# Scoobadood/TSDF

Hardware: AMD Instinct MI355X
Metric: Mvoxels/s integrate + Mrays/s raycast, 512^3 grid, 640x480 depth; 1/2/4/8 GPU (higher is better)
Workload: dtype f32; 1 GPU; configs[2]: 512^3 TSDF over 3000 mm, synthetic TUM-surrogate stream (200-frame trajectory, seed 0x5EED0003), 640x480 uint16 depth, bilateral(30,4.5) + integrate + raycast + normals per frame; parallelism=zslab1, depth_tile_maxima=left by the bilateral filter's launch, ranks=1

## Files before the change

### include/tsdf_amd.h

```cpp
#ifndef TSDF_AMD_H
#define TSDF_AMD_H

#include <stddef.h>
#include <stdint.h>

#ifdef __cplusplus
extern "C" {
#endif

#define TSDF_OK 0
#define TSDF_ERR_INVALID 1
#define TSDF_ERR_DEVICE 2
#define TSDF_ERR_NOMEM 3

typedef struct tsdf_volume tsdf_volume;
typedef struct tsdf_bilateral tsdf_bilateral;
typedef struct tsdf_icp tsdf_icp;

typedef struct tsdf_volume_info {
    uint32_t size[3];
    uint32_t z_begin, z_end;
    uint32_t z_store_begin, z_store_end;
    float physical_size[3];
    float voxel_size[3];
// ... 31 lines not shown
                            tsdf_volume **out);
int tsdf_volume_destroy(tsdf_volume *volume);
int tsdf_volume_set_stream(tsdf_volume *volume, void *hip_stream);
int tsdf_volume_stream(const tsdf_volume *volume, void **hip_stream);
int tsdf_volume_synchronize(const tsdf_volume *volume);
int tsdf_volume_clear(tsdf_volume *volume);
int tsdf_volume_get_info(const tsdf_volume *volume, tsdf_volume_info *info);
int tsdf_volume_set_offset(tsdf_volume *volume, float ox, float oy, float oz);

int tsdf_volume_set_header(tsdf_volume *volume, const float offset[3], float truncation_distance,
                           float max_weight, const float global_translation[3],
                           const float global_rotation[3]);

int tsdf_volume_distances(const tsdf_volume *volume, float **device_ptr);
int tsdf_volume_mark_dirty(tsdf_volume *volume);
int tsdf_volume_weights(const tsdf_volume *volume, float **device_ptr);
int tsdf_volume_weight_storage(const tsdf_volume *volume, int *bits_per_weight, int *pinned);
int tsdf_volume_set_weight_storage(tsdf_volume *volume, int bits_per_weight);
int tsdf_selftest_count_division(uint32_t b_begin, uint32_t b_end, unsigned long long *mismatches);
int tsdf_selftest_bilateral_chain_taps(size_t n, const float *w, const uint32_t *v4, const float *s, float *s_f32, float *s_f64,
                                       uint8_t *certified);
int tsdf_selftest_bilateral_chain_image(float sigma_colour, float sigma_space, const void *image, int bits_per_pixel, int width, int height,
                                        void *filtered, unsigned long long counts[4]);
int tsdf_volume_deformation(tsdf_volume *volume, tsdf_deformation_node **device_ptr);
int tsdf_volume_set_distance_data(tsdf_volume *volume, const float *host);
int tsdf_volume_set_weight_data(tsdf_volume *volume, const float *host);
int tsdf_volume_set_deformation(tsdf_volume *volume, const tsdf_deformation_node *host);
int tsdf_volume_deform_points(const tsdf_volume *volume, int num_points, float *host_points);
int tsdf_volume_deform_points_device(const tsdf_volume *volume, int num_points, float *device_points);
int tsdf_volume_get_distance_data(const tsdf_volume *volume, float *host);
int tsdf_volume_get_weight_data(const tsdf_volume *volume, float *host);
int tsdf_volume_get_deformation_planes(const tsdf_volume *volume, uint32_t plane_begin, uint32_t plane_count,
                                       tsdf_deformation_node *host);
int tsdf_volume_set_offset_at_clear(tsdf_volume *volume, const float offset_at_clear[3]);

int tsdf_integrate(tsdf_volume *volume, const uint16_t *host_depth, uint32_t width, uint32_t height,
                   const float pose[16], const float inv_pose[16], const float k[9], const float kinv[9]);
int tsdf_integrate_device(tsdf_volume *volume, const uint16_t *device_depth, uint32_t width,
                          uint32_t height, const float pose[16], const float inv_pose[16],
                          const float k[9], const float kinv[9]);
int tsdf_integrate_device_tiles(tsdf_volume *volume, const uint16_t *device_depth, uint32_t width,
                                uint32_t height, const float pose[16], const float inv_pose[16],
                                const float k[9], const float kinv[9], const uint16_t *device_tile_max);
int tsdf_integrate_prepare_device_tiles(tsdf_volume *volume, const uint16_t *device_depth, uint32_t width,
                                        uint32_t height, const float pose[16], const float inv_pose[16],
                                        const float k[9], const float kinv[9], const uint16_t *device_tile_max,
// ... 316 lines not shown
```

### tsdf_amd/_capi.py

```python
import ctypes as C
import os

_HERE = os.path.dirname(os.path.abspath(__file__))
LIB_PATH = os.environ.get("TSDF_HIP_LIB") or os.path.join(_HERE, "lib", "libtsdf_hip.so")

TSDF_OK, TSDF_ERR_INVALID, TSDF_ERR_DEVICE, TSDF_ERR_NOMEM = 0, 1, 2, 3
TSDF_FIELD_UNIT_GRADIENT = 1
TSDF_RAYS_BAND_ONLY = 1
TSDF_MESH_NORMALS, TSDF_MESH_COLOURS = 1, 2
TSDF_MESH_KEEP_LARGEST = 1
TSDF_SMOOTH_PIN_BOUNDARY, TSDF_SMOOTH_NORMALS = 1, 2
TSDF_ESDF_FILL_UNKNOWN = 1
TSDF_SCENE_FLOW_DEFORMED = 1


class TsdfError(RuntimeError):
    """A C-ABI call failed with TSDF_ERR_DEVICE / TSDF_ERR_NOMEM."""


class VolumeInfo(C.Structure):
    _fields_ = [("size", C.c_uint32 * 3), ("z_begin", C.c_uint32), ("z_end", C.c_uint32),
                ("z_store_begin", C.c_uint32), ("z_store_end", C.c_uint32),
                ("physical_size", C.c_float * 3), ("voxel_size", C.c_float * 3), ("offset", C.c_float * 3),
                ("offset_at_clear", C.c_float * 3), ("truncation_distance", C.c_float),
# ... 60 lines not shown
    "tsdf_stream_synchronize": (_i, [_vp]),
    "tsdf_volume_create": (_i, [_u32, _u32, _u32, _f, _f, _f, C.POINTER(_vp)]),
    "tsdf_volume_create_slab": (_i, [_u32, _u32, _u32, _f, _f, _f, _u32, _u32, C.POINTER(_vp)]),
    "tsdf_volume_destroy": (_i, [_vp]),
    "tsdf_volume_set_stream": (_i, [_vp, _vp]),
    "tsdf_volume_stream": (_i, [_vp, C.POINTER(_vp)]),
    "tsdf_volume_synchronize": (_i, [_vp]),
    "tsdf_volume_clear": (_i, [_vp]),
    "tsdf_volume_get_info": (_i, [_vp, C.POINTER(VolumeInfo)]),
    "tsdf_volume_set_offset": (_i, [_vp, _f, _f, _f]),
    "tsdf_volume_set_header": (_i, [_vp, _fp, _f, _f, _fp, _fp]),
    "tsdf_volume_mark_dirty": (_i, [_vp]),
    "tsdf_volume_distances": (_i, [_vp, C.POINTER(_vp)]),
    "tsdf_volume_weights": (_i, [_vp, C.POINTER(_vp)]),
    "tsdf_volume_weight_storage": (_i, [_vp, C.POINTER(_i), C.POINTER(_i)]),
    "tsdf_volume_last_raycast_kind": (_i, [_vp, C.POINTER(_i)]),
    "tsdf_volume_last_cell_list": (_i, [_vp, C.POINTER(C.c_uint32)]),
    "tsdf_volume_set_weight_storage": (_i, [_vp, _i]),
    "tsdf_volume_set_weight_cap": (_i, [_vp, C.c_uint32]),
    "tsdf_volume_weight_cap": (_i, [_vp, C.POINTER(C.c_uint32)]),
    "tsdf_selftest_count_division": (_i, [_u32, _u32, C.POINTER(C.c_uint64)]),
    "tsdf_selftest_bilateral_chain_taps": (_i, [C.c_size_t, _vp, _vp, _vp, _vp, _vp, _vp]),
    "tsdf_selftest_bilateral_chain_image": (_i, [_f, _f, _vp, _i, _i, _i, _vp, C.POINTER(C.c_uint64)]),
    "tsdf_volume_deformation": (_i, [_vp, C.POINTER(_vp)]),
    "tsdf_volume_set_distance_data": (_i, [_vp, _vp]),
    "tsdf_volume_set_weight_data": (_i, [_vp, _vp]),
    "tsdf_volume_set_deformation": (_i, [_vp, _vp]),
    "tsdf_volume_get_distance_data": (_i, [_vp, _vp]),
    "tsdf_measure_copy_bandwidth": (_i, [C.c_size_t, _i, _vp, C.POINTER(C.c_double)]),
    "tsdf_measure_update_bandwidth": (_i, [_i, _vp, C.POINTER(C.c_double)]),
    "tsdf_volume_get_weight_data": (_i, [_vp, _vp]),
    "tsdf_volume_get_deformation_planes": (_i, [_vp, C.c_uint32, C.c_uint32, _vp]),
    "tsdf_volume_set_offset_at_clear": (_i, [_vp, _vp]),
    "tsdf_integrate": (_i, [_vp, _vp, _u32, _u32, _fp, _fp, _fp, _fp]),
    "tsdf_integrate_device": (_i, [_vp, _vp, _u32, _u32, _fp, _fp, _fp, _fp]),
    "tsdf_deintegrate": (_i, [_vp, _vp, _u32, _u32, _fp, _fp, _fp, _fp]),
    "tsdf_deintegrate_device": (_i, [_vp, _vp, _u32, _u32, _fp, _fp, _fp, _fp]),
    "tsdf_integrate_device_tiles": (_i, [_vp, _vp, _u32, _u32, _fp, _fp, _fp, _fp, _vp]),
    "tsdf_integrate_prepare_device_tiles": (_i, [_vp, _vp, _u32, _u32, _fp, _fp, _fp, _fp, _vp, _vp]),
    "tsdf_integrate_discard_prepared": (_i, [_vp]),
    "tsdf_volume_set_timing": (_i, [_vp, _i]),
    "tsdf_volume_kernel_time": (_i, [_vp, _i, C.POINTER(C.c_uint32), C.POINTER(C.c_float)]),
    "tsdf_volume_set_counting": (_i, [_vp, _i]),
    "tsdf_volume_last_updated_voxels": (_i, [_vp, C.POINTER(C.c_uint64)]),
    "tsdf_volume_last_distance_stores": (_i, [_vp, C.POINTER(C.c_uint64)]),
    "tsdf_volume_enable_colour": (_i, [_vp, _i]),
# ... 190 lines not shown
```

### tsdf_amd/csrc/raycast.hip

```cpp
#include <algorithm>
#include <cmath>
#include <cstdlib>

#include "common.hpp"
#include "raycast_sample.hpp"
#include "field_sample.hpp"

namespace tsdf {

__device__ inline bool can_intersect_in_dimension(float space_min, float space_max, float origin, float direction,
                                                  float &near_t, float &far_t) {
    bool can_intersect = true;
    if (direction == 0) {
        if (origin < space_min || origin > space_max) can_intersect = false;
    } else {
        float dmin = (space_min - origin) / direction;
        float dmax = (space_max - origin) / direction;
        if (dmin > dmax) {
            float t = dmin;
            dmin = dmax;
            dmax = t;
        }
        if (dmin > near_t) near_t = dmin;
        if (dmax < far_t) far_t = dmax;
        if (near_t > far_t) can_intersect = false;
        else if (far_t < 0) can_intersect = false;
    }
    return can_intersect;
}
// ... 202 lines not shown
    }

    k_first = k_lo;
    if (SLAB && k_end > 0) {
        const float za = ((float)rp.own_lo - 2.0f) * g.vs.z, zb = ((float)rp.own_hi + 2.0f) * g.vs.z;
        if (dir.z != 0.0f) {
            const float r = __builtin_amdgcn_rcpf(dir.z);
            const float t0 = (za - sz) * r, t1 = (zb - sz) * r;
            const float ta = fminf(t0, t1), tb = fmaxf(t0, t1);
            const float ka = floorf(ta * __builtin_amdgcn_rcpf(step_size)) - 3.0f;
            const float kb = ceilf(tb * __builtin_amdgcn_rcpf(step_size)) + 3.0f;
            if (ka > (float)k_first) k_first = (int)fminf(ka, (float)kMaxSamples);
            if (kb < (float)k_end) k_end = (int)fmaxf(kb, 0.0f);
        } else if (sz < za || sz > zb) {
            k_end = 0;
        }
    }
}

__device__ inline SkipCtx make_skip_ctx(const Geom &g, float step_size) {
    SkipCtx sc;
    sc.inv_vx = __builtin_amdgcn_rcpf(g.vs.x); sc.inv_vy = __builtin_amdgcn_rcpf(g.vs.y); sc.inv_vz = __builtin_amdgcn_rcpf(g.vs.z);
    sc.inv_step = __builtin_amdgcn_rcpf(step_size);
    sc.eps = fmaxf(1.0e-3f, 2.0e-6f * (float)max(g.X, max(g.Y, g.Z)));
    sc.tx = sc.ty = sc.tz = INFINITY;
    sc.su = sc.sv = sc.sw = INFINITY;
    sc.posx = sc.posy = sc.posz = 1.0f;
    sc.skip_ok = false;
    return sc;
}

struct TailQueue {
    uint2 *entries;
    uint32_t *count;
    uint32_t trip_budget;
    uint32_t lanes;
    uint64_t *best;
    int piece_min;
    const uint32_t *order;
    uint8_t *heavy;
    uint32_t heavy_passes;
};
constexpr uint32_t kTailSignals = 4 + 2 * 256;
constexpr uint32_t kNoHit = 0xffffffffu;
constexpr uint32_t kNoSlot = 0xffffffffu;
__host__ __device__ inline uint32_t ray_range_of_slot(uint32_t z, uint32_t nz, uint32_t order) {
    return order == 0 ? z : order == 1 ? nz - 1u - z : (z == 0 ? nz - 1u : z == 1 ? 0u : nz - z);
// ... 875 lines not shown
                          nullptr);
}

int tsdf_volume_cast_rays_colour_device(const tsdf_volume *v, uint64_t n, const float *device_origins, const float *device_directions,
                                        const float *device_t_max, float *device_points, float *device_t, float *device_normals,
                                        uint8_t *device_rgb) {
    int rc = cast_rays_colour_check(v, n, device_origins, device_directions, device_points, device_t, device_normals, device_rgb);
    if (rc != TSDF_OK) return rc;
    if (n == 0) return TSDF_OK;
    rc = cast_rays(const_cast<tsdf_volume *>(v), n, device_origins, device_directions, device_t_max, device_points, device_t, device_normals);
    if (rc != TSDF_OK) return rc;
    return cast_rays_colour(v, n, device_points, device_rgb);
}

int tsdf_volume_cast_rays_colour(const tsdf_volume *cv, uint64_t n, const float *host_origins, const float *host_directions,
                                 const float *host_t_max, float *host_points, float *host_t, float *host_normals, uint8_t *host_rgb) {
    const int rc0 = cast_rays_colour_check(cv, n, host_origins, host_directions, host_points, host_t, host_normals, host_rgb);
    if (rc0 != TSDF_OK) return rc0;
    if (n == 0) return TSDF_OK;
    return cast_rays_host(const_cast<tsdf_volume *>(cv), n, host_origins, host_directions, host_t_max, host_points, host_t, host_normals,
                          host_rgb);
}

}
```

### tsdf_amd/csrc/raycast_cells.hpp

```cpp

struct RayRecord {
    float near_t;
    uint32_t k_range;
};
static_assert(sizeof(RayRecord) == 8, "one 8-byte load");

struct CellCast {
    RayRecord *rays;
    uint2 *bricks;
    uint32_t *n_bricks;
    uint32_t *n_bricks_host;
    uint32_t pairs_per_task;
    uint32_t *depth_hist;
    uint2 *unsorted;
    float depth0, depth_scale;
    const float *dist;
    uint64_t *best;
};
constexpr uint32_t kCellTasks = 1u << 31, kShellTasks = 1u << 30;
constexpr uint32_t kDepthBins = 256;
__device__ inline uint32_t depth_bin(const CellCast &cc, const EntryParams &ep, const Geom &g, uint32_t coords) {
    const float mid = 0.5f * ((float)kBrick + 1.5f);
    const float wx = ((float)((coords & 1023u) * kBrick) + mid) * g.vs.x + ep.offset.x, wy = ((float)(((coords >> 10) & 1023u) * kBrick) + mid) * g.vs.y + ep.offset.y,
                wz = ((float)((coords >> 20) * kBrick) + mid) * g.vs.z + ep.offset.z;
    const float d = ep.r[2][0] * wx + ep.r[2][1] * wy + ep.r[2][2] * wz + ep.r[2][3];
    const float b = (d - cc.depth0) * cc.depth_scale;
    return b > 0.0f ? (b < (float)(kDepthBins - 1u) ? (uint32_t)b : kDepthBins - 1u) : 0u;
}
constexpr uint32_t kMaxParts = 1024, kPartsRoom = 1024;
__host__ __device__ inline size_t cell_list_capacity(size_t n_bricks) { return n_bricks + (size_t)kPartsRoom * ((n_bricks + 1023) / 1024); }

struct PixelBox {
    int u0, v0, w, h;
};
template <bool HULL = true>
__device__ inline bool project_box(const EntryParams &ep, float lox, float loy, float loz, float hix, float hiy, float hiz, PixelBox &pb) {
    const float mx = 0.5f * (lox + hix) + ep.offset.x, my = 0.5f * (loy + hiy) + ep.offset.y, mz = 0.5f * (loz + hiz) + ep.offset.z;
    const float ccx = ep.r[0][0] * mx + ep.r[0][1] * my + ep.r[0][2] * mz + ep.r[0][3];
    const float ccy = ep.r[1][0] * mx + ep.r[1][1] * my + ep.r[1][2] * mz + ep.r[1][3];
    const float ccz = ep.r[2][0] * mx + ep.r[2][1] * my + ep.r[2][2] * mz + ep.r[2][3];
    const float ext[3] = {hix - lox, hiy - loy, hiz - loz};
    const float hz = 0.5f * ((fabsf(ep.r[2][0] * ext[0]) + fabsf(ep.r[2][1] * ext[1])) + fabsf(ep.r[2][2] * ext[2]));
    const float zslack = 1.0e-5f * (((fabsf(ep.r[2][0] * mx) + fabsf(ep.r[2][1] * my)) + fabsf(ep.r[2][2] * mz)) + fabsf(ep.r[2][3])) + 1.0e-5f * hz;
    const float zmin = ccz - hz - zslack, zmax = ccz + hz + zslack;
    if (!(ccx == ccx && ccy == ccy && zmin == zmin && zmax == zmax) || fabsf(ccx) == INFINITY || fabsf(ccy) == INFINITY || zmax == INFINITY || zmin == -INFINITY) {
        pb.u0 = 0; pb.v0 = 0; pb.w = (int)ep.width; pb.h = (int)ep.height;
        return true;
    }
    if (zmax < ep.z_clip) return false;
    float a0, a1, b0, b1;
    const float kMargin = 0.05f;
    if (HULL && zmin > ep.z_near) {
        float umin = INFINITY, umax = -INFINITY, vmin = INFINITY, vmax = -INFINITY;
#pragma unroll
        for (int c = 0; c < 8; c++) {
            const float wx = ((c & 1) ? hix : lox) + ep.offset.x, wy = ((c & 2) ? hiy : loy) + ep.offset.y, wz = ((c & 4) ? hiz : loz) + ep.offset.z;
            const float cx = ep.r[0][0] * wx + ep.r[0][1] * wy + ep.r[0][2] * wz + ep.r[0][3];
            const float cy = ep.r[1][0] * wx + ep.r[1][1] * wy + ep.r[1][2] * wz + ep.r[1][3];
            const float cz = fmaxf(ep.r[2][0] * wx + ep.r[2][1] * wy + ep.r[2][2] * wz + ep.r[2][3], 0.5f * ep.z_near);
            const float rz = __builtin_amdgcn_rcpf(cz);
            const float u = (ep.k[0][0] * cx + ep.k[0][1] * cy + ep.k[0][2] * cz) * rz, w = (ep.k[1][0] * cx + ep.k[1][1] * cy + ep.k[1][2] * cz) * rz;
            umin = fminf(umin, u); umax = fmaxf(umax, u);
            vmin = fminf(vmin, w); vmax = fmaxf(vmax, w);
        }
        a0 = ceilf(umin - kMargin); a1 = floorf(umax + kMargin); b0 = ceilf(vmin - kMargin); b1 = floorf(vmax + kMargin);
    } else {
        const float us = 0.5f * (float)ep.width, vs_ = 0.5f * (float)ep.height;
        const float dlo = fmaxf(zmin, ep.z_clip), rhi = 1.0f / (zmax * 1.0001f), rlo = dlo > 0.0f ? 1.0001f / dlo : INFINITY;
        auto side = [&](const float *kr, float centre, float &lo_, float &hi_) {
            const float t0 = kr[0] * ccx, t1 = kr[1] * ccy, t2 = kr[2] * ccz, t3 = centre * ccz;
            const float fc = ((t0 + t1) + t2) - t3;
            float h = 0.0f;
#pragma unroll
            for (int a_ = 0; a_ < 3; a_++) {
                const float ex_ = ep.r[0][a_] * ext[a_], ey_ = ep.r[1][a_] * ext[a_], ez_ = ep.r[2][a_] * ext[a_];
                h += 0.5f * fabsf(((kr[0] * ex_ + kr[1] * ey_) + kr[2] * ez_) - centre * ez_);
            }
            const float slack = 1.0e-5f * ((((fabsf(t0) + fabsf(t1)) + fabsf(t2)) + fabsf(t3)) + h) + (fabsf(kr[0]) + fabsf(kr[1]) + fabsf(kr[2]) + centre) * zslack;
            const float fmin_ = fc - h - slack, fmax_ = fc + h + slack;
            lo_ = fmin_ > 0.0f ? fmin_ * rhi : (dlo > 0.0f ? fmin_ * rlo : -INFINITY);
            hi_ = fmax_ < 0.0f ? fmax_ * rhi : (dlo > 0.0f ? fmax_ * rlo : INFINITY);
        };
        float ul, uh, vl, vh;
        side(ep.k[0], us, ul, uh);
        side(ep.k[1], vs_, vl, vh);
        a0 = ceilf(us + ul - kMargin); a1 = floorf(us + uh + kMargin); b0 = ceilf(vs_ + vl - kMargin); b1 = floorf(vs_ + vh + kMargin);
    }
    const float wmax = (float)(ep.width - 1u), hmax = (float)(ep.height - 1u);
    if (!(a0 <= a1 && b0 <= b1) || a1 < 0.0f || b1 < 0.0f || a0 > wmax || b0 > hmax) return false;
    pb.u0 = (int)fmaxf(a0, 0.0f); pb.v0 = (int)fmaxf(b0, 0.0f);
    pb.w = (int)fminf(a1, wmax) - pb.u0 + 1; pb.h = (int)fminf(b1, hmax) - pb.v0 + 1;
    return true;
}
template <int CTRL, int ROW_MASK>
__device__ inline uint32_t dpp_or_zero(uint32_t v) {
    return (uint32_t)__builtin_amdgcn_update_dpp(0, (int)v, CTRL, ROW_MASK, 0xf, false);
}
__device__ inline uint32_t wave_scan_add(uint32_t v) {
    v += dpp_or_zero<0x111, 0xf>(v);
    v += dpp_or_zero<0x112, 0xf>(v);
    v += dpp_or_zero<0x114, 0xf>(v);
    v += dpp_or_zero<0x118, 0xf>(v);
    v += dpp_or_zero<0x142, 0xa>(v);
    v += dpp_or_zero<0x143, 0xc>(v);
    return v;
}
__device__ inline uint32_t wave_scan_max(uint32_t v) {
    v = max(v, dpp_or_zero<0x111, 0xf>(v));
    v = max(v, dpp_or_zero<0x112, 0xf>(v));
    v = max(v, dpp_or_zero<0x114, 0xf>(v));
    v = max(v, dpp_or_zero<0x118, 0xf>(v));
    v = max(v, dpp_or_zero<0x142, 0xa>(v));
    v = max(v, dpp_or_zero<0x143, 0xc>(v));
    return v;
}
template <bool SLAB>
// ... 307 lines not shown
                }
            }
        }
    }
}

#ifndef TSDF_CELLS_WAVES
#define TSDF_CELLS_WAVES 4
#endif
#ifndef TSDF_CELLS_SCAN_DECODE
#define TSDF_CELLS_SCAN_DECODE 1
#endif
template <bool SLAB, bool FASTDIV>
#if TSDF_CELLS_WAVES
__attribute__((amdgpu_waves_per_eu(TSDF_CELLS_WAVES, TSDF_CELLS_WAVES)))
#endif
__global__ __launch_bounds__(256) void cast_cells_kernel(const float *__restrict__ dist, const Geom g, const RayParams rp, const EntryParams ep,
                                                         const OccGrid occ, const float *__restrict__ t_table, const CellCast cc,
                                                         uint64_t *__restrict__ best) {
    __shared__ __attribute__((aligned(16))) float T[kTableLen];
    __shared__ float corner[4][128];
    __shared__ __attribute__((aligned(16))) int box_of[4][64][4];
    __shared__ int prefix[4][64];
#if TSDF_CELLS_SCAN_DECODE
    __shared__ uint32_t mark[4][64];
    mark[threadIdx.x >> 6][threadIdx.x & 63u] = 0u;
    uint32_t round = 0u;
#endif
    static_assert(kTableLen % 4 == 0, "the table in 16-byte pieces");
    for (int i = (int)threadIdx.x; i < kTableLen / 4; i += 256) reinterpret_cast<float4 *>(T)[i] = reinterpret_cast<const float4 *>(t_table)[i];
    const uint32_t n_bricks = *cc.n_bricks;
    if (cc.n_bricks_host && blockIdx.x == 0 && threadIdx.x == 0) *cc.n_bricks_host = n_bricks;
    static_assert(sizeof(box_of) >= 256 * sizeof(uint2), "a shell workgroup's list of bricks");
    if (blockIdx.x < kShellWorkgroups) {
        __syncthreads();
        cast_shell_bricks<SLAB, FASTDIV>(dist, g, rp, ep, T, cc, best, n_bricks, reinterpret_cast<uint2 *>(&box_of[0][0][0]), reinterpret_cast<uint32_t *>(&prefix[0][0]));
        return;
    }
    const uint32_t wave = threadIdx.x >> 6, lane = threadIdx.x & 63u;
    const float step_size = t_table[1];
    const TriConst &tc = rp.tc;
    const SkipCtx sc = make_skip_ctx(g, step_size);
    const float e = sc.eps;
    const size_t plane = (size_t)g.X * g.Y;
    const float ex = (1.0f + 2.0f * e) * g.vs.x, ey = (1.0f + 2.0f * e) * g.vs.y, ez = (1.0f + 2.0f * e) * g.vs.z;
    float nu_[3], nv_[3], nz_[3];
#pragma unroll
    for (int a_ = 0; a_ < 3; a_++) {
        const float ext = a_ == 0 ? ex : a_ == 1 ? ey : ez;
        const float cxa = ep.r[0][a_] * ext, cya = ep.r[1][a_] * ext, cza = ep.r[2][a_] * ext;
        nu_[a_] = ep.k[0][0] * cxa + ep.k[0][1] * cya + ep.k[0][2] * cza;
        nv_[a_] = ep.k[1][0] * cxa + ep.k[1][1] * cya + ep.k[1][2] * cza;
        nz_[a_] = cza;
    }
    const float half_dz = 0.5f * ((fabsf(nz_[0]) + fabsf(nz_[1])) + fabsf(nz_[2]));
    __syncthreads();
    auto wave_sync = [] {
        __builtin_amdgcn_fence(__ATOMIC_RELEASE, "wavefront");
        __builtin_amdgcn_s_waitcnt(0xc07f);
        __builtin_amdgcn_wave_barrier();
        __builtin_amdgcn_fence(__ATOMIC_ACQUIRE, "wavefront");
    };
    auto offset_of = [&](uint32_t i) { return (size_t)(i / 25u) * plane + (size_t)((i / 5u) % 5u) * g.X + (i % 5u); };
    const size_t off_a = offset_of(lane), off_b = offset_of(min(lane + 64u, 124u));
    auto brick_voxels = [&](uint2 entry_, float &va, float &vb) {
        va = vb = 0.0f;
        if (!(entry_.x & kCellTasks)) return;
        const uint32_t bx_ = entry_.y & 1023u, by_ = (entry_.y >> 10) & 1023u, bz_ = entry_.y >> 20;
        if (bx_ * kBrick + kBrick < g.X && by_ * kBrick + kBrick < g.Y && bz_ * kBrick >= g.z_store_begin && bz_ * kBrick + kBrick < g.z_store_end) {
            const float *first = dist + (plane * (bz_ * kBrick - g.z_store_begin) + (size_t)g.X * (by_ * kBrick) + bx_ * kBrick);
            va = first[off_a];
            vb = first[off_b];
            return;
        }
        auto voxel = [&](uint32_t i) {
            const uint32_t cx = i % 5u, cy = (i / 5u) % 5u, cz = i / 25u;
            const uint32_t vx = min(bx_ * kBrick + cx, g.X - 1u), vy = min(by_ * kBrick + cy, g.Y - 1u);
            const uint32_t vz = min(max(bz_ * kBrick + cz, g.z_store_begin), g.z_store_end - 1u);
            return dist[plane * (vz - g.z_store_begin) + (size_t)g.X * vy + vx];
        };
        va = voxel(lane);
        if (lane + 64u < 125u) vb = voxel(lane + 64u);
    };
    const uint32_t n_waves = (gridDim.x - kShellWorkgroups) * 4u;
    uint32_t ei = (blockIdx.x - kShellWorkgroups) * 4u + wave;
    uint2 entry_next = ei < n_bricks ? cc.bricks[ei] : make_uint2(0u, 0u);
    float va_next, vb_next;
    brick_voxels(entry_next, va_next, vb_next);
    for (; ei < n_bricks; ei += n_waves) {
        const uint2 entry2 = entry_next;
        const uint32_t entry = entry2.x;
        const float va = va_next, vb = vb_next;
        entry_next = ei + n_waves < n_bricks ? cc.bricks[ei + n_waves] : make_uint2(0u, 0u);
        brick_voxels(entry_next, va_next, vb_next);
        const uint32_t bx = entry2.y & 1023u, by = (entry2.y >> 10) & 1023u, bz = entry2.y >> 20;
        const uint32_t x0 = bx * kBrick, y0 = by * kBrick, z0 = bz * kBrick;
        wave_sync();
        corner[wave][lane] = va;
        corner[wave][lane + 64u] = vb;
        wave_sync();
        const uint32_t cx = lane & 3u, cy = (lane >> 2) & 3u, cz = lane >> 4;
        const uint32_t lx = x0 + cx, ly = y0 + cy, lz = z0 + cz;
        bool mixed = false;
        if (entry & kCellTasks) {
            bool valid = lx + 1u < g.X && ly + 1u < g.Y && lz + 1u < g.Z && lz >= g.z_store_begin && lz + 1u < g.z_store_end;
            if (SLAB) valid = valid && lz >= rp.own_lo && lz < rp.own_hi;
            const float *c = &corner[wave][cx + 5u * cy + 25u * cz];
            const bool positive = fminf(fminf(fminf(c[0], c[1]), fminf(c[5], c[6])), fminf(fminf(c[25], c[26]), fminf(c[30], c[31]))) > kCellPositive;
            mixed = valid && !positive;
        }
        PixelBox pb = {0, 0, 0, 0};
        if (mixed) {
            const float wx = ((float)lx + 1.0f) * g.vs.x + ep.offset.x, wy = ((float)ly + 1.0f) * g.vs.y + ep.offset.y, wz = ((float)lz + 1.0f) * g.vs.z + ep.offset.z;
            const float ccx = ep.r[0][0] * wx + ep.r[0][1] * wy + ep.r[0][2] * wz + ep.r[0][3];
            const float ccy = ep.r[1][0] * wx + ep.r[1][1] * wy + ep.r[1][2] * wz + ep.r[1][3];
            const float ccz = ep.r[2][0] * wx + ep.r[2][1] * wy + ep.r[2][2] * wz + ep.r[2][3];
            const float zmin = ccz - half_dz;
            if (zmin > ep.z_near) {
                const float rz = __builtin_amdgcn_rcpf(ccz), rm = __builtin_amdgcn_rcpf(zmin);
                const float uc = (ep.k[0][0] * ccx + ep.k[0][1] * ccy + ep.k[0][2] * ccz) * rz, vc = (ep.k[1][0] * ccx + ep.k[1][1] * ccy + ep.k[1][2] * ccz) * rz;
                const float su = 0.5f * ((fabsf(nu_[0] - uc * nz_[0]) + fabsf(nu_[1] - uc * nz_[1])) + fabsf(nu_[2] - uc * nz_[2]));
                const float sv = 0.5f * ((fabsf(nv_[0] - vc * nz_[0]) + fabsf(nv_[1] - vc * nz_[1])) + fabsf(nv_[2] - vc * nz_[2]));
                const float hu = su * rm * 1.0001f + 0.05f, hv = sv * rm * 1.0001f + 0.05f;
                const float a0 = fmaxf(ceilf(uc - hu), 0.0f), a1 = fminf(floorf(uc + hu), (float)(ep.width - 1u));
                const float b0 = fmaxf(ceilf(vc - hv), 0.0f), b1 = fminf(floorf(vc + hv), (float)(ep.height - 1u));
                mixed = a0 <= a1 && b0 <= b1;
                if (mixed) { pb.u0 = (int)a0; pb.v0 = (int)b0; pb.w = (int)a1 - (int)a0 + 1; pb.h = (int)b1 - (int)b0 + 1; }
            } else {
                const float clx = ((float)lx + 0.5f - e) * g.vs.x, chx = ((float)lx + 1.5f + e) * g.vs.x;
                const float cly = ((float)ly + 0.5f - e) * g.vs.y, chy = ((float)ly + 1.5f + e) * g.vs.y;
                const float clz = ((float)lz + 0.5f - e) * g.vs.z, chz = ((float)lz + 1.5f + e) * g.vs.z;
                mixed = project_box<false>(ep, clx, cly, clz, chx, chy, chz, pb);
            }
        }
        if (lane == 0) { RAY_MIX(32); }
        if (mixed) { RAY_MIX(33); }
#if TSDF_CELLS_SCAN_DECODE
        const int n_mine = mixed ? pb.w * pb.h : 0, incl = (int)wave_scan_add((uint32_t)n_mine);
        const int n_pairs = __builtin_amdgcn_readlane(incl, 63);
        const int first_mine = incl - n_mine;
        if (mixed) {
            box_of[wave][lane][0] = pb.u0; box_of[wave][lane][1] = pb.v0; box_of[wave][lane][2] = pb.w; box_of[wave][lane][3] = first_mine;
        }
#else
        int n_mine = mixed ? pb.w * pb.h : 0, incl = n_mine;
        for (int o = 1; o < 64; o <<= 1) {
            const int up = __shfl_up(incl, o);
            if ((int)lane >= o) incl += up;
        }
        const int n_pairs = __shfl(incl, 63);
        prefix[wave][lane] = incl - n_mine;
        if (mixed) {
            box_of[wave][lane][0] = pb.u0; box_of[wave][lane][1] = pb.v0; box_of[wave][lane][2] = pb.w; box_of[wave][lane][3] = pb.h;
        }
        wave_sync();
#endif
// ... 107 lines not shown
```

Measured before the change: 644,400 Mvoxels/s.

## Precompute per-view cell box projection constants in shared memory for raycast cells

Moves the per-cell pixel-box projection into a shared header and precomputes an affine form of the projection (numerators and depth as linear functions of cell index, plus rigorous error bounds) once per workgroup into shared memory. Each lane then evaluates the box with a few FMAs instead of a full world-to-camera transform. The table load into LDS is split into register staging so the constant setup overlaps the global loads. It adds a host selftest entry point and changes rounding slack, so box extents may shift slightly.

```diff
diff --git a/include/tsdf_amd.h b/include/tsdf_amd.h
--- a/include/tsdf_amd.h
+++ b/include/tsdf_amd.h
@@ -77,6 +77,9 @@
                                        uint8_t *certified);
 int tsdf_selftest_bilateral_chain_image(float sigma_colour, float sigma_space, const void *image, int bits_per_pixel, int width, int height,
                                         void *filtered, unsigned long long counts[4]);
+int tsdf_selftest_cell_boxes(const float *r, const float *k, const float *voxel_size, const float *offset, const uint32_t *grid,
+                             uint32_t width, uint32_t height, float z_clip, float z_near, size_t n, const uint32_t *cells, int corners_only,
+                             int32_t *boxes, uint8_t *seen);
 int tsdf_volume_deformation(tsdf_volume *volume, tsdf_deformation_node **device_ptr);
 int tsdf_volume_set_distance_data(tsdf_volume *volume, const float *host);
 int tsdf_volume_set_weight_data(tsdf_volume *volume, const float *host);
diff --git a/tsdf_amd/_capi.py b/tsdf_amd/_capi.py
--- a/tsdf_amd/_capi.py
+++ b/tsdf_amd/_capi.py
@@ -106,6 +106,7 @@
     "tsdf_selftest_count_division": (_i, [_u32, _u32, C.POINTER(C.c_uint64)]),
     "tsdf_selftest_bilateral_chain_taps": (_i, [C.c_size_t, _vp, _vp, _vp, _vp, _vp, _vp]),
     "tsdf_selftest_bilateral_chain_image": (_i, [_f, _f, _vp, _i, _i, _i, _vp, C.POINTER(C.c_uint64)]),
+    "tsdf_selftest_cell_boxes": (_i, [_vp, _vp, _vp, _vp, _vp, _u32, _u32, _f, _f, C.c_size_t, _vp, _i, _vp, _vp]),
     "tsdf_volume_deformation": (_i, [_vp, C.POINTER(_vp)]),
     "tsdf_volume_set_distance_data": (_i, [_vp, _vp]),
     "tsdf_volume_set_weight_data": (_i, [_vp, _vp]),
diff --git a/tsdf_amd/csrc/cell_boxes.hpp b/tsdf_amd/csrc/cell_boxes.hpp
--- /dev/null
+++ b/tsdf_amd/csrc/cell_boxes.hpp
@@ -0,0 +1,200 @@
+#pragma once
+#include <cmath>
+#include <cstdint>
+
+#if defined(__HIPCC__) || defined(__CUDACC__)
+#define TSDF_BOX_HD __host__ __device__
+#else
+#define TSDF_BOX_HD
+#endif
+
+namespace tsdf {
+
+TSDF_BOX_HD inline float box_rcp(float x) {
+#if defined(__HIP_DEVICE_COMPILE__)
+    return __builtin_amdgcn_rcpf(x);
+#else
+    return 1.0f / x;
+#endif
+}
+
+TSDF_BOX_HD inline float cell_guard_eps(uint32_t x, uint32_t y, uint32_t z) {
+    const uint32_t m = x > y ? (x > z ? x : z) : (y > z ? y : z);
+    return fmaxf(1.0e-3f, 2.0e-6f * (float)m);
+}
+
+struct PixelBox {
+    int u0, v0, w, h;
+};
+template <bool HULL = true, class V>
+TSDF_BOX_HD inline bool project_box(const V &ep, float lox, float loy, float loz, float hix, float hiy, float hiz, PixelBox &pb) {
+    const float mx = 0.5f * (lox + hix) + ep.offset.x, my = 0.5f * (loy + hiy) + ep.offset.y, mz = 0.5f * (loz + hiz) + ep.offset.z;
+    const float ccx = ep.r[0][0] * mx + ep.r[0][1] * my + ep.r[0][2] * mz + ep.r[0][3];
+    const float ccy = ep.r[1][0] * mx + ep.r[1][1] * my + ep.r[1][2] * mz + ep.r[1][3];
+    const float ccz = ep.r[2][0] * mx + ep.r[2][1] * my + ep.r[2][2] * mz + ep.r[2][3];
+    const float ext[3] = {hix - lox, hiy - loy, hiz - loz};
+    const float hz = 0.5f * ((fabsf(ep.r[2][0] * ext[0]) + fabsf(ep.r[2][1] * ext[1])) + fabsf(ep.r[2][2] * ext[2]));
+    const float zslack = 1.0e-5f * (((fabsf(ep.r[2][0] * mx) + fabsf(ep.r[2][1] * my)) + fabsf(ep.r[2][2] * mz)) + fabsf(ep.r[2][3])) + 1.0e-5f * hz;
+    const float zmin = ccz - hz - zslack, zmax = ccz + hz + zslack;
+    if (!(ccx == ccx && ccy == ccy && zmin == zmin && zmax == zmax) || fabsf(ccx) == INFINITY || fabsf(ccy) == INFINITY || zmax == INFINITY || zmin == -INFINITY) {
+        pb.u0 = 0; pb.v0 = 0; pb.w = (int)ep.width; pb.h = (int)ep.height;
+        return true;
+    }
+    if (zmax < ep.z_clip) return false;
+    float a0, a1, b0, b1;
+    const float kMargin = 0.05f;
+    if (HULL && zmin > ep.z_near) {
+        float umin = INFINITY, umax = -INFINITY, vmin = INFINITY, vmax = -INFINITY;
+#pragma unroll
+        for (int c = 0; c < 8; c++) {
+            const float wx = ((c & 1) ? hix : lox) + ep.offset.x, wy = ((c & 2) ? hiy : loy) + ep.offset.y, wz = ((c & 4) ? hiz : loz) + ep.offset.z;
+            const float cx = ep.r[0][0] * wx + ep.r[0][1] * wy + ep.r[0][2] * wz + ep.r[0][3];
+            const float cy = ep.r[1][0] * wx + ep.r[1][1] * wy + ep.r[1][2] * wz + ep.r[1][3];
+            const float cz = fmaxf(ep.r[2][0] * wx + ep.r[2][1] * wy + ep.r[2][2] * wz + ep.r[2][3], 0.5f * ep.z_near);
+            const float rz = box_rcp(cz);
+            const float u = (ep.k[0][0] * cx + ep.k[0][1] * cy + ep.k[0][2] * cz) * rz, w = (ep.k[1][0] * cx + ep.k[1][1] * cy + ep.k[1][2] * cz) * rz;
+            umin = fminf(umin, u); umax = fmaxf(umax, u);
+            vmin = fminf(vmin, w); vmax = fmaxf(vmax, w);
+        }
+        a0 = ceilf(umin - kMargin); a1 = floorf(umax + kMargin); b0 = ceilf(vmin - kMargin); b1 = floorf(vmax + kMargin);
+    } else {
+        const float us = 0.5f * (float)ep.width, vs_ = 0.5f * (float)ep.height;
+        const float dlo = fmaxf(zmin, ep.z_clip), rhi = 1.0f / (zmax * 1.0001f), rlo = dlo > 0.0f ? 1.0001f / dlo : INFINITY;
+        auto side = [&](const float *kr, float centre, float &lo_, float &hi_) {
+            const float t0 = kr[0] * ccx, t1 = kr[1] * ccy, t2 = kr[2] * ccz, t3 = centre * ccz;
+            const float fc = ((t0 + t1) + t2) - t3;
+            float h = 0.0f;
+#pragma unroll
+            for (int a_ = 0; a_ < 3; a_++) {
+                const float ex_ = ep.r[0][a_] * ext[a_], ey_ = ep.r[1][a_] * ext[a_], ez_ = ep.r[2][a_] * ext[a_];
+                h += 0.5f * fabsf(((kr[0] * ex_ + kr[1] * ey_) + kr[2] * ez_) - centre * ez_);
+            }
+            const float slack = 1.0e-5f * ((((fabsf(t0) + fabsf(t1)) + fabsf(t2)) + fabsf(t3)) + h) + (fabsf(kr[0]) + fabsf(kr[1]) + fabsf(kr[2]) + centre) * zslack;
+            const float fmin_ = fc - h - slack, fmax_ = fc + h + slack;
+            lo_ = fmin_ > 0.0f ? fmin_ * rhi : (dlo > 0.0f ? fmin_ * rlo : -INFINITY);
+            hi_ = fmax_ < 0.0f ? fmax_ * rhi : (dlo > 0.0f ? fmax_ * rlo : INFINITY);
+        };
+        float ul, uh, vl, vh;
+        side(ep.k[0], us, ul, uh);
+        side(ep.k[1], vs_, vl, vh);
+        a0 = ceilf(us + ul - kMargin); a1 = floorf(us + uh + kMargin); b0 = ceilf(vs_ + vl - kMargin); b1 = floorf(vs_ + vh + kMargin);
+    }
+    const float wmax = (float)(ep.width - 1u), hmax = (float)(ep.height - 1u);
+    if (!(a0 <= a1 && b0 <= b1) || a1 < 0.0f || b1 < 0.0f || a0 > wmax || b0 > hmax) return false;
+    pb.u0 = (int)fmaxf(a0, 0.0f); pb.v0 = (int)fmaxf(b0, 0.0f);
+    pb.w = (int)fminf(a1, wmax) - pb.u0 + 1; pb.h = (int)fminf(b1, hmax) - pb.v0 + 1;
+    return true;
+}
+
+struct CellBoxFast {
+    float nu[4], nv[4], dz[4];
+    float lim[4];
+    float edge[4];
+};
+struct CellBoxF3 {
+    float x, y, z;
+};
+struct alignas(16) CellBoxConsts {
+    CellBoxFast fast;
+    float r[3][4];
+    float k[2][3];
+    CellBoxF3 vs, offset;
+    float e, z_clip, z_near;
+    uint32_t width, height;
+};
+static_assert(sizeof(CellBoxFast) == 80 && sizeof(CellBoxConsts) % 16 == 0, "rows of 16 bytes");
+
+template <class V>
+TSDF_BOX_HD inline void cell_box_consts(CellBoxConsts &c, const V &ep, float vsx, float vsy, float vsz, uint32_t gx, uint32_t gy, uint32_t gz, float e) {
+    const double vs[3] = {vsx, vsy, vsz}, size[3] = {(double)gx, (double)gy, (double)gz};
+    const double off[3] = {ep.offset.x, ep.offset.y, ep.offset.z};
+    double t[3], m[3][3], a_[3], reach[3];
+#pragma unroll
+    for (int a = 0; a < 3; a++) reach[a] = __builtin_fma(size[a] + 1.0, vs[a], fabs(off[a]));
+#pragma unroll
+    for (int j = 0; j < 3; j++) {
+        t[j] = ep.r[j][3];
+        a_[j] = fabs((double)ep.r[j][3]);
+#pragma unroll
+        for (int a = 0; a < 3; a++) {
+            m[j][a] = (double)ep.r[j][a] * vs[a];
+            t[j] = __builtin_fma((double)ep.r[j][a], off[a] + vs[a], t[j]);
+            a_[j] = __builtin_fma(fabs((double)ep.r[j][a]), reach[a], a_[j]);
+        }
+    }
+    double b[3], old[2];
+#pragma unroll
+    for (int i = 0; i < 2; i++) {
+        float *row = i == 0 ? c.fast.nu : c.fast.nv;
+        const double k0 = ep.k[i][0], k1 = ep.k[i][1], k2 = ep.k[i][2];
+        const double t_ = __builtin_fma(k2, t[2], __builtin_fma(k1, t[1], k0 * t[0]));
+        row[0] = (float)t_;
+        b[i] = fabs(t_);
+#pragma unroll
+        for (int a = 0; a < 3; a++) {
+            const double p = __builtin_fma(k2, m[2][a], __builtin_fma(k1, m[1][a], k0 * m[0][a]));
+            row[1 + a] = (float)p;
+            b[i] = __builtin_fma(size[a], fabs(p), b[i]);
+        }
+        old[i] = __builtin_fma(fabs(k2), a_[2], __builtin_fma(fabs(k1), a_[1], fabs(k0) * a_[0]));
+    }
+    c.fast.dz[0] = (float)t[2];
+    b[2] = fabs(t[2]);
+    double edges_z = 0.0;
+#pragma unroll
+    for (int a = 0; a < 3; a++) {
+        c.fast.dz[1 + a] = (float)m[2][a];
+        b[2] = __builtin_fma(size[a], fabs(m[2][a]), b[2]);
+        edges_z += fabs(m[2][a]);
+    }
+    const double u = 1.0 / 16777216.0, up = 1.0 + 2.0 * u;
+    const double grown = 1.0 + 2.0 * (double)e, grow_z = u * __builtin_fma(5.0, b[2], 11.0 * a_[2]);
+    c.fast.lim[0] = (float)(__builtin_fma(0.5 * grown, edges_z, grow_z) * up);
+    c.fast.lim[1] = ep.z_near;
+    c.fast.lim[2] = (float)(0.5 * grown * 1.0001);
+    c.fast.lim[3] = (float)(2.0 * up * u * __builtin_fma(13.0, b[2], 11.0 * a_[2]));
+    c.fast.edge[0] = (float)(2.0 * up * u * __builtin_fma(5.0, b[0], 11.0 * old[0]));
+    c.fast.edge[1] = (float)(2.0 * up * u * __builtin_fma(5.0, b[1], 11.0 * old[1]));
+    c.fast.edge[2] = (float)(ep.width - 1u);
+    c.fast.edge[3] = (float)(ep.height - 1u);
+    for (int j = 0; j < 3; j++)
+        for (int a = 0; a < 4; a++) c.r[j][a] = ep.r[j][a];
+    for (int j = 0; j < 2; j++)
+        for (int a = 0; a < 3; a++) c.k[j][a] = ep.k[j][a];
+    c.vs = {vsx, vsy, vsz};
+    c.offset = {ep.offset.x, ep.offset.y, ep.offset.z};
+    c.e = e;
+    c.z_clip = ep.z_clip;
+    c.z_near = ep.z_near;
+    c.width = ep.width;
+    c.height = ep.height;
+}
+
+TSDF_BOX_HD inline bool cell_box_front(const CellBoxFast &f, uint32_t lx, uint32_t ly, uint32_t lz, PixelBox &pb, bool &near) {
+    const float fx = (float)lx, fy = (float)ly, fz = (float)lz;
+    const float nu = __builtin_fmaf(fz, f.nu[3], __builtin_fmaf(fy, f.nu[2], __builtin_fmaf(fx, f.nu[1], f.nu[0])));
+    const float nv = __builtin_fmaf(fz, f.nv[3], __builtin_fmaf(fy, f.nv[2], __builtin_fmaf(fx, f.nv[1], f.nv[0])));
+    const float d = __builtin_fmaf(fz, f.dz[3], __builtin_fmaf(fy, f.dz[2], __builtin_fmaf(fx, f.dz[1], f.dz[0])));
+    const float zmin = d - f.lim[0];
+    near = !(zmin > f.lim[1]);
+    if (near) return false;
+    const float rz = box_rcp(d), rm = box_rcp(zmin) * f.lim[2];
+    const float uc = nu * rz, vc = nv * rz;
+    const float su = ((__builtin_fmaf(fabsf(uc), f.lim[3], f.edge[0]) + fabsf(__builtin_fmaf(-uc, f.dz[1], f.nu[1]))) + fabsf(__builtin_fmaf(-uc, f.dz[2], f.nu[2]))) + fabsf(__builtin_fmaf(-uc, f.dz[3], f.nu[3]));
+    const float sv = ((__builtin_fmaf(fabsf(vc), f.lim[3], f.edge[1]) + fabsf(__builtin_fmaf(-vc, f.dz[1], f.nv[1]))) + fabsf(__builtin_fmaf(-vc, f.dz[2], f.nv[2]))) + fabsf(__builtin_fmaf(-vc, f.dz[3], f.nv[3]));
+    const float hu = __builtin_fmaf(su, rm, 0.05f), hv = __builtin_fmaf(sv, rm, 0.05f);
+    const float a0 = fmaxf(ceilf(uc - hu), 0.0f), a1 = fminf(floorf(uc + hu), f.edge[2]);
+    const float b0 = fmaxf(ceilf(vc - hv), 0.0f), b1 = fminf(floorf(vc + hv), f.edge[3]);
+    if (!(a0 <= a1 && b0 <= b1)) return false;
+    pb.u0 = (int)a0; pb.v0 = (int)b0; pb.w = (int)a1 - (int)a0 + 1; pb.h = (int)b1 - (int)b0 + 1;
+    return true;
+}
+TSDF_BOX_HD inline bool cell_box_near(const CellBoxConsts &c, uint32_t lx, uint32_t ly, uint32_t lz, PixelBox &pb) {
+    const float e = c.e;
+    const float clx = ((float)lx + 0.5f - e) * c.vs.x, chx = ((float)lx + 1.5f + e) * c.vs.x;
+    const float cly = ((float)ly + 0.5f - e) * c.vs.y, chy = ((float)ly + 1.5f + e) * c.vs.y;
+    const float clz = ((float)lz + 0.5f - e) * c.vs.z, chz = ((float)lz + 1.5f + e) * c.vs.z;
+    return project_box<false>(c, clx, cly, clz, chx, chy, chz, pb);
+}
+
+}
diff --git a/tsdf_amd/csrc/raycast.hip b/tsdf_amd/csrc/raycast.hip
--- a/tsdf_amd/csrc/raycast.hip
+++ b/tsdf_amd/csrc/raycast.hip
@@ -5,6 +5,7 @@
 #include "common.hpp"
 #include "raycast_sample.hpp"
 #include "field_sample.hpp"
+#include "cell_boxes.hpp"
 
 namespace tsdf {
 
@@ -253,7 +254,7 @@
     SkipCtx sc;
     sc.inv_vx = __builtin_amdgcn_rcpf(g.vs.x); sc.inv_vy = __builtin_amdgcn_rcpf(g.vs.y); sc.inv_vz = __builtin_amdgcn_rcpf(g.vs.z);
     sc.inv_step = __builtin_amdgcn_rcpf(step_size);
-    sc.eps = fmaxf(1.0e-3f, 2.0e-6f * (float)max(g.X, max(g.Y, g.Z)));
+    sc.eps = cell_guard_eps(g.X, g.Y, g.Z);
     sc.tx = sc.ty = sc.tz = INFINITY;
     sc.su = sc.sv = sc.sw = INFINITY;
     sc.posx = sc.posy = sc.posz = 1.0f;
@@ -1175,4 +1176,37 @@
                           host_rgb);
 }
 
-}
+int tsdf_selftest_cell_boxes(const float *r, const float *k, const float *voxel_size, const float *offset, const uint32_t *grid,
+                             uint32_t width, uint32_t height, float z_clip, float z_near, size_t n, const uint32_t *cells, int corners_only,
+                             int32_t *boxes, uint8_t *seen) {
+    TSDF_REQUIRE(r && k && voxel_size && offset && grid && cells && boxes && seen, "tsdf_selftest_cell_boxes: null pointer");
+    TSDF_REQUIRE(width >= 1 && height >= 1 && grid[0] >= 2 && grid[1] >= 2 && grid[2] >= 2, "tsdf_selftest_cell_boxes: empty image or grid");
+    TSDF_REQUIRE(z_near > 0.0f && z_near >= z_clip && z_clip >= 0.0f, "tsdf_selftest_cell_boxes: 0 <= z_clip <= z_near, 0 < z_near");
+    EntryParams ep{};
+    for (int j = 0; j < 3; j++)
+        for (int a = 0; a < 4; a++) ep.r[j][a] = r[4 * j + a];
+    for (int j = 0; j < 2; j++)
+        for (int a = 0; a < 3; a++) ep.k[j][a] = k[3 * j + a];
+    ep.vs = {voxel_size[0], voxel_size[1], voxel_size[2]};
+    ep.offset = {offset[0], offset[1], offset[2]};
+    ep.width = width;
+    ep.height = height;
+    ep.z_clip = z_clip;
+    ep.z_near = z_near;
+    CellBoxConsts c;
+    cell_box_consts(c, ep, voxel_size[0], voxel_size[1], voxel_size[2], grid[0], grid[1], grid[2], cell_guard_eps(grid[0], grid[1], grid[2]));
+    for (size_t i = 0; i < n; i++) {
+        const uint32_t lx = cells[3 * i], ly = cells[3 * i + 1], lz = cells[3 * i + 2];
+        TSDF_REQUIRE(lx + 1u < grid[0] && ly + 1u < grid[1] && lz + 1u < grid[2], "tsdf_selftest_cell_boxes: cell %zu is not a cell of the grid", i);
+        PixelBox pb = {0, 0, 0, 0};
+        bool near = true, any = false;
+        if (!corners_only) any = cell_box_front(c.fast, lx, ly, lz, pb, near);
+        if (near) any = cell_box_near(c, lx, ly, lz, pb);
+        if (!any) pb = {0, 0, 0, 0};
+        boxes[4 * i] = pb.u0; boxes[4 * i + 1] = pb.v0; boxes[4 * i + 2] = pb.w; boxes[4 * i + 3] = pb.h;
+        seen[i] = (uint8_t)((any ? 1 : 0) | (near ? 2 : 0));
+    }
+    return TSDF_OK;
+}
+
+}
diff --git a/tsdf_amd/csrc/raycast_cells.hpp b/tsdf_amd/csrc/raycast_cells.hpp
--- a/tsdf_amd/csrc/raycast_cells.hpp
+++ b/tsdf_amd/csrc/raycast_cells.hpp
@@ -30,68 +30,6 @@
 constexpr uint32_t kMaxParts = 1024, kPartsRoom = 1024;
 __host__ __device__ inline size_t cell_list_capacity(size_t n_bricks) { return n_bricks + (size_t)kPartsRoom * ((n_bricks + 1023) / 1024); }
 
-struct PixelBox {
-    int u0, v0, w, h;
-};
-template <bool HULL = true>
-__device__ inline bool project_box(const EntryParams &ep, float lox, float loy, float loz, float hix, float hiy, float hiz, PixelBox &pb) {
-    const float mx = 0.5f * (lox + hix) + ep.offset.x, my = 0.5f * (loy + hiy) + ep.offset.y, mz = 0.5f * (loz + hiz) + ep.offset.z;
-    const float ccx = ep.r[0][0] * mx + ep.r[0][1] * my + ep.r[0][2] * mz + ep.r[0][3];
-    const float ccy = ep.r[1][0] * mx + ep.r[1][1] * my + ep.r[1][2] * mz + ep.r[1][3];
-    const float ccz = ep.r[2][0] * mx + ep.r[2][1] * my + ep.r[2][2] * mz + ep.r[2][3];
-    const float ext[3] = {hix - lox, hiy - loy, hiz - loz};
-    const float hz = 0.5f * ((fabsf(ep.r[2][0] * ext[0]) + fabsf(ep.r[2][1] * ext[1])) + fabsf(ep.r[2][2] * ext[2]));
-    const float zslack = 1.0e-5f * (((fabsf(ep.r[2][0] * mx) + fabsf(ep.r[2][1] * my)) + fabsf(ep.r[2][2] * mz)) + fabsf(ep.r[2][3])) + 1.0e-5f * hz;
-    const float zmin = ccz - hz - zslack, zmax = ccz + hz + zslack;
-    if (!(ccx == ccx && ccy == ccy && zmin == zmin && zmax == zmax) || fabsf(ccx) == INFINITY || fabsf(ccy) == INFINITY || zmax == INFINITY || zmin == -INFINITY) {
-        pb.u0 = 0; pb.v0 = 0; pb.w = (int)ep.width; pb.h = (int)ep.height;
-        return true;
-    }
-    if (zmax < ep.z_clip) return false;
-    float a0, a1, b0, b1;
-    const float kMargin = 0.05f;
-    if (HULL && zmin > ep.z_near) {
-        float umin = INFINITY, umax = -INFINITY, vmin = INFINITY, vmax = -INFINITY;
-#pragma unroll
-        for (int c = 0; c < 8; c++) {
-            const float wx = ((c & 1) ? hix : lox) + ep.offset.x, wy = ((c & 2) ? hiy : loy) + ep.offset.y, wz = ((c & 4) ? hiz : loz) + ep.offset.z;
-            const float cx = ep.r[0][0] * wx + ep.r[0][1] * wy + ep.r[0][2] * wz + ep.r[0][3];
-            const float cy = ep.r[1][0] * wx + ep.r[1][1] * wy + ep.r[1][2] * wz + ep.r[1][3];
-            const float cz = fmaxf(ep.r[2][0] * wx + ep.r[2][1] * wy + ep.r[2][2] * wz + ep.r[2][3], 0.5f * ep.z_near);
-            const float rz = __builtin_amdgcn_rcpf(cz);
-            const float u = (ep.k[0][0] * cx + ep.k[0][1] * cy + ep.k[0][2] * cz) * rz, w = (ep.k[1][0] * cx + ep.k[1][1] * cy + ep.k[1][2] * cz) * rz;
-            umin = fminf(umin, u); umax = fmaxf(umax, u);
-            vmin = fminf(vmin, w); vmax = fmaxf(vmax, w);
-        }
-        a0 = ceilf(umin - kMargin); a1 = floorf(umax + kMargin); b0 = ceilf(vmin - kMargin); b1 = floorf(vmax + kMargin);
-    } else {
-        const float us = 0.5f * (float)ep.width, vs_ = 0.5f * (float)ep.height;
-        const float dlo = fmaxf(zmin, ep.z_clip), rhi = 1.0f / (zmax * 1.0001f), rlo = dlo > 0.0f ? 1.0001f / dlo : INFINITY;
-        auto side = [&](const float *kr, float centre, float &lo_, float &hi_) {
-            const float t0 = kr[0] * ccx, t1 = kr[1] * ccy, t2 = kr[2] * ccz, t3 = centre * ccz;
-            const float fc = ((t0 + t1) + t2) - t3;
-            float h = 0.0f;
-#pragma unroll
-            for (int a_ = 0; a_ < 3; a_++) {
-                const float ex_ = ep.r[0][a_] * ext[a_], ey_ = ep.r[1][a_] * ext[a_], ez_ = ep.r[2][a_] * ext[a_];
-                h += 0.5f * fabsf(((kr[0] * ex_ + kr[1] * ey_) + kr[2] * ez_) - centre * ez_);
-            }
-            const float slack = 1.0e-5f * ((((fabsf(t0) + fabsf(t1)) + fabsf(t2)) + fabsf(t3)) + h) + (fabsf(kr[0]) + fabsf(kr[1]) + fabsf(kr[2]) + centre) * zslack;
-            const float fmin_ = fc - h - slack, fmax_ = fc + h + slack;
-            lo_ = fmin_ > 0.0f ? fmin_ * rhi : (dlo > 0.0f ? fmin_ * rlo : -INFINITY);
-            hi_ = fmax_ < 0.0f ? fmax_ * rhi : (dlo > 0.0f ? fmax_ * rlo : INFINITY);
-        };
-        float ul, uh, vl, vh;
-        side(ep.k[0], us, ul, uh);
-        side(ep.k[1], vs_, vl, vh);
-        a0 = ceilf(us + ul - kMargin); a1 = floorf(us + uh + kMargin); b0 = ceilf(vs_ + vl - kMargin); b1 = floorf(vs_ + vh + kMargin);
-    }
-    const float wmax = (float)(ep.width - 1u), hmax = (float)(ep.height - 1u);
-    if (!(a0 <= a1 && b0 <= b1) || a1 < 0.0f || b1 < 0.0f || a0 > wmax || b0 > hmax) return false;
-    pb.u0 = (int)fmaxf(a0, 0.0f); pb.v0 = (int)fmaxf(b0, 0.0f);
-    pb.w = (int)fminf(a1, wmax) - pb.u0 + 1; pb.h = (int)fminf(b1, hmax) - pb.v0 + 1;
-    return true;
-}
 template <int CTRL, int ROW_MASK>
 __device__ inline uint32_t dpp_or_zero(uint32_t v) {
     return (uint32_t)__builtin_amdgcn_update_dpp(0, (int)v, CTRL, ROW_MASK, 0xf, false);
@@ -445,13 +383,30 @@
     __shared__ float corner[4][128];
     __shared__ __attribute__((aligned(16))) int box_of[4][64][4];
     __shared__ int prefix[4][64];
+    __shared__ CellBoxConsts view_c;
 #if TSDF_CELLS_SCAN_DECODE
     __shared__ uint32_t mark[4][64];
     mark[threadIdx.x >> 6][threadIdx.x & 63u] = 0u;
     uint32_t round = 0u;
 #endif
     static_assert(kTableLen % 4 == 0, "the table in 16-byte pieces");
-    for (int i = (int)threadIdx.x; i < kTableLen / 4; i += 256) reinterpret_cast<float4 *>(T)[i] = reinterpret_cast<const float4 *>(t_table)[i];
+    constexpr int kTableTurns = (kTableLen / 4 + 255) / 256;
+    float4 table_part[kTableTurns];
+#pragma unroll
+    for (int j = 0; j < kTableTurns; j++) {
+        const int i = (int)threadIdx.x + 256 * j;
+        table_part[j] = reinterpret_cast<const float4 *>(t_table)[min(i, kTableLen / 4 - 1)];
+    }
+    if (blockIdx.x >= kShellWorkgroups && threadIdx.x == 0) cell_box_consts(view_c, ep, g.vs.x, g.vs.y, g.vs.z, g.X, g.Y, g.Z, cell_guard_eps(g.X, g.Y, g.Z));
+#pragma unroll
+    for (int j = 0; j < kTableTurns; j++) {
+        asm volatile("" : "+v"(table_part[j].x), "+v"(table_part[j].y), "+v"(table_part[j].z), "+v"(table_part[j].w));
+    }
+#pragma unroll
+    for (int j = 0; j < kTableTurns; j++) {
+        const int i = (int)threadIdx.x + 256 * j;
+        if (256 * j + 255 < kTableLen / 4 || i < kTableLen / 4) reinterpret_cast<float4 *>(T)[i] = table_part[j];
+    }
     const uint32_t n_bricks = *cc.n_bricks;
     if (cc.n_bricks_host && blockIdx.x == 0 && threadIdx.x == 0) *cc.n_bricks_host = n_bricks;
     static_assert(sizeof(box_of) >= 256 * sizeof(uint2), "a shell workgroup's list of bricks");
@@ -466,17 +421,6 @@
     const SkipCtx sc = make_skip_ctx(g, step_size);
     const float e = sc.eps;
     const size_t plane = (size_t)g.X * g.Y;
-    const float ex = (1.0f + 2.0f * e) * g.vs.x, ey = (1.0f + 2.0f * e) * g.vs.y, ez = (1.0f + 2.0f * e) * g.vs.z;
-    float nu_[3], nv_[3], nz_[3];
-#pragma unroll
-    for (int a_ = 0; a_ < 3; a_++) {
-        const float ext = a_ == 0 ? ex : a_ == 1 ? ey : ez;
-        const float cxa = ep.r[0][a_] * ext, cya = ep.r[1][a_] * ext, cza = ep.r[2][a_] * ext;
-        nu_[a_] = ep.k[0][0] * cxa + ep.k[0][1] * cya + ep.k[0][2] * cza;
-        nv_[a_] = ep.k[1][0] * cxa + ep.k[1][1] * cya + ep.k[1][2] * cza;
-        nz_[a_] = cza;
-    }
-    const float half_dz = 0.5f * ((fabsf(nz_[0]) + fabsf(nz_[1])) + fabsf(nz_[2]));
     __syncthreads();
     auto wave_sync = [] {
         __builtin_amdgcn_fence(__ATOMIC_RELEASE, "wavefront");
@@ -521,6 +465,9 @@
         wave_sync();
         corner[wave][lane] = va;
         corner[wave][lane + 64u] = vb;
+        CellBoxFast bf;
+#pragma unroll
+        for (int i = 0; i < 5; i++) reinterpret_cast<float4 *>(&bf)[i] = reinterpret_cast<const float4 *>(&view_c.fast)[i];
         wave_sync();
         const uint32_t cx = lane & 3u, cy = (lane >> 2) & 3u, cz = lane >> 4;
         const uint32_t lx = x0 + cx, ly = y0 + cy, lz = z0 + cz;
@@ -534,27 +481,9 @@
         }
         PixelBox pb = {0, 0, 0, 0};
         if (mixed) {
-            const float wx = ((float)lx + 1.0f) * g.vs.x + ep.offset.x, wy = ((float)ly + 1.0f) * g.vs.y + ep.offset.y, wz = ((float)lz + 1.0f) * g.vs.z + ep.offset.z;
-            const float ccx = ep.r[0][0] * wx + ep.r[0][1] * wy + ep.r[0][2] * wz + ep.r[0][3];
-            const float ccy = ep.r[1][0] * wx + ep.r[1][1] * wy + ep.r[1][2] * wz + ep.r[1][3];
-            const float ccz = ep.r[2][0] * wx + ep.r[2][1] * wy + ep.r[2][2] * wz + ep.r[2][3];
-            const float zmin = ccz - half_dz;
-            if (zmin > ep.z_near) {
-                const float rz = __builtin_amdgcn_rcpf(ccz), rm = __builtin_amdgcn_rcpf(zmin);
-                const float uc = (ep.k[0][0] * ccx + ep.k[0][1] * ccy + ep.k[0][2] * ccz) * rz, vc = (ep.k[1][0] * ccx + ep.k[1][1] * ccy + ep.k[1][2] * ccz) * rz;
-                const float su = 0.5f * ((fabsf(nu_[0] - uc * nz_[0]) + fabsf(nu_[1] - uc * nz_[1])) + fabsf(nu_[2] - uc * nz_[2]));
-                const float sv = 0.5f * ((fabsf(nv_[0] - vc * nz_[0]) + fabsf(nv_[1] - vc * nz_[1])) + fabsf(nv_[2] - vc * nz_[2]));
-                const float hu = su * rm * 1.0001f + 0.05f, hv = sv * rm * 1.0001f + 0.05f;
-                const float a0 = fmaxf(ceilf(uc - hu), 0.0f), a1 = fminf(floorf(uc + hu), (float)(ep.width - 1u));
-                const float b0 = fmaxf(ceilf(vc - hv), 0.0f), b1 = fminf(floorf(vc + hv), (float)(ep.height - 1u));
-                mixed = a0 <= a1 && b0 <= b1;
-                if (mixed) { pb.u0 = (int)a0; pb.v0 = (int)b0; pb.w = (int)a1 - (int)a0 + 1; pb.h = (int)b1 - (int)b0 + 1; }
-            } else {
-                const float clx = ((float)lx + 0.5f - e) * g.vs.x, chx = ((float)lx + 1.5f + e) * g.vs.x;
-                const float cly = ((float)ly + 0.5f - e) * g.vs.y, chy = ((float)ly + 1.5f + e) * g.vs.y;
-                const float clz = ((float)lz + 0.5f - e) * g.vs.z, chz = ((float)lz + 1.5f + e) * g.vs.z;
-                mixed = project_box<false>(ep, clx, cly, clz, chx, chy, chz, pb);
-            }
+            bool near;
+            mixed = cell_box_front(bf, lx, ly, lz, pb, near);
+            if (near) mixed = cell_box_near(view_c, lx, ly, lz, pb);
         }
         if (lane == 0) { RAY_MIX(32); }
         if (mixed) { RAY_MIX(33); }
```

Measured after the change: 654,800 Mvoxels/s (median of 6 runs). 1.6% higher.
